# maciejkula/spotlight

Measured on NVIDIA H100. Metric: interactions/sec (BPR MF, 1Mx100Kx64), higher is better.
Workload: dtype f32

## Files before the change

spotlight_b200/csrc/mf.cu:

```cuda
#include <stdlib.h>

#include "segindex.cuh"

namespace {

constexpr int MF_THREADS = 256;

struct MfDev {
    int64_t B;
    int64_t NB;
    int64_t T;
    const int64_t* users; const int64_t* items; const int64_t* negs;
    int32_t loss; int32_t n_neg;
    int64_t U, I; int32_t D;
    float* Wu; float* Wi; float* bu; float* bi;
    float* loss_out; float* pos_out; float* neg_out;
    int32_t* t_a; int32_t* t_b; float* t_g;
    float* partial; int32_t* done;
    int32_t* err;
    SegIndex seg;
    int32_t grad_mode;
    float* dWu; float* dWi; float* dbu; float* dbi;
    int64_t* urows; float* gWu; float* gbu;
    int64_t* irows; float* gWi; float* gbi;
// ... 1076 lines not shown
        SLB_LAUNCH_CHECK("mf_fwd_kernel");
    }
    if (phases & 2) {
        seg_scan_launch(a.seg, a.U, st);
        SLB_LAUNCH_CHECK("seg_scan_kernel");
    }
    int fgrid = static_cast<int>((2 * B + 255) / 256);
    if (fgrid > sms * 8) fgrid = sms * 8;
    if (phases & 4) {
        mf_fill_kernel<<<fgrid, 256, 0, st>>>(a);
        SLB_LAUNCH_CHECK("mf_fill_kernel");
        seg_sort_long_kernel<<<SEG_LONG_CTAS, 256, 0, st>>>(a.seg);
        SLB_LAUNCH_CHECK("seg_sort_long_kernel");
    }
    int64_t bwant = (2 * B + groups - 1) / groups;
    int bgrid = static_cast<int>(bwant < static_cast<int64_t>(sms) * 8 ? bwant : static_cast<int64_t>(sms) * 8);
    const bool bsmall = 2 * B < static_cast<int64_t>(sms) * 24 * 32;
    const int bti = bsmall ? 8 : 32;
    const int64_t tw = ((2 * B + bti - 1) / bti + 3) / 4;
    const int tgrid = static_cast<int>(tw < static_cast<int64_t>(sms) * 16 ? tw : static_cast<int64_t>(sms) * 16);
    const int blpr = lpr;
#define BWD_TILE(MODE)                                                                               \
    if (bsmall) { DISPATCH_LPR3(blpr, mf_bwd_tile_kernel, MODE, 8, tgrid, MF_TILE_THREADS, st, a); } \
    else { DISPATCH_LPR3(blpr, mf_bwd_tile_kernel, MODE, 32, tgrid, MF_TILE_THREADS, st, a); }
    if (x->opt == SLB_OPT_NONE || x->opt == SLB_OPT_ADAM) {
        if (phases & 8) {
            BWD_TILE(0);
            SLB_LAUNCH_CHECK("mf_bwd_tile_kernel");
            launch_long<0>(lpr, st, a);
            SLB_LAUNCH_CHECK("mf_bwd_long_kernel");
        }
        if (x->opt == SLB_OPT_ADAM && (phases & 16)) {
            AdamDev o = {x->beta1, x->beta2, x->one_minus_beta1, x->one_minus_beta2, x->eps, x->weight_decay, x->adam_sched,
                         static_cast<int32_t>(x->adam_step + step_idx)};
            DISPATCH_LPR(lpr, mf_adam_apply_kernel, bgrid, MF_THREADS, st, a, o, x->state2_Wu, x->state2_Wi,
                         x->state2_bu, x->state2_bi, x->last_u, x->last_i);
            SLB_LAUNCH_CHECK("mf_adam_apply_kernel");
        }
    } else {
        if (phases & 8) {
            BWD_TILE(1);
            SLB_LAUNCH_CHECK("mf_bwd_tile_kernel<items>");
            launch_long<1>(lpr, st, a);
            SLB_LAUNCH_CHECK("mf_bwd_long_kernel<items>");
#if BWD_BULK
            if (lpr == 16 && a.D == 64 && !bsmall) {
                auto kern = mf_bwd_tile_kernel<16, 2, 32, true>;
                constexpr int BULK_SMEM = (MF_TILE_THREADS / 32) * 32 * 2 * 256;
                static bool configured = false;
                if (!configured) {
                    cudaFuncSetAttribute(kern, cudaFuncAttributeMaxDynamicSharedMemorySize, BULK_SMEM);
                    configured = true;
                }
                kern<<<tgrid, MF_TILE_THREADS, BULK_SMEM, st>>>(a);
            } else
#endif
            { BWD_TILE(2); }
            SLB_LAUNCH_CHECK("mf_bwd_tile_kernel<users+opt>");
            launch_long<2>(lpr, st, a);
            SLB_LAUNCH_CHECK("mf_bwd_long_kernel<users+opt>");
        }
        if ((phases & 16) && !x->opt_users_only) {
            DISPATCH_LPR2(lpr, mf_apply_kernel, 1, bgrid, MF_THREADS, st, a);
            SLB_LAUNCH_CHECK("mf_apply_kernel<items>");
        }
    }
    return SLB_OK;
}


struct V2Layout {
    PlanDev plan[2];
    StepV2 st;
    size_t bytes;
};

V2Layout v2_layout(void* base, int64_t B, int64_t U, int64_t I, int D) {
    WsCarver ws(base);
    V2Layout l;
    const int64_t R = U + I;
    const int64_t Rpad = (R + SEG_SCAN_TILE - 1) / SEG_SCAN_TILE * SEG_SCAN_TILE;
    l.st.done = ws.take<int32_t>(8);
    int32_t* cnt[2] = {ws.take<int32_t>(Rpad), ws.take<int32_t>(Rpad)};
    for (int k = 0; k < 2; ++k) {
        PlanDev& p = l.plan[k];
        SegIndex& s = p.seg;
        s.R = R;
        s.Rpad = Rpad;
        s.ntiles = s.Rpad / SEG_SCAN_TILE;
        s.Tmax = 3 * B;
        s.cnt = cnt[k];
        s.off = ws.take<int32_t>(s.Rpad);
        s.sid = ws.take<int32_t>(s.Rpad);
        s.status = ws.take<unsigned long long>(s.ntiles);
        s.ticket = ws.take<int32_t>(8);
        s.totals = s.ticket + 4;
        s.seg_row = ws.take<int32_t>(3 * B + 1);
        s.seg_start = ws.take<int32_t>(3 * B + 2);
        s.long_list = ws.take<int32_t>(3 * B / 16 + 2);
        s.members = nullptr; s.long_tmp = nullptr; s.long_bits = nullptr; s.long_words = 0;
        s.long_cap = 0;
        p.mu = ws.take<URec>(B + 1);
        p.mi = ws.take<IRec>(2 * B + 1);
        p.mu_tmp = ws.take<URec>(B + 1);
        p.mi_tmp = ws.take<IRec>(2 * B + 1);
        p.words = (2 * B + 31) / 32;
        p.bits = ws.take<uint32_t>(static_cast<size_t>(SEG_LONG_CTAS) * 2 * p.words);
        p.B = B; p.U = U; p.I = I;
        p.err = nullptr; p.users = nullptr; p.items = nullptr; p.negs = nullptr; p.ratings = nullptr;
    }
    l.st.t_g = ws.take<float>(2 * B);
    l.st.stash = ws.take<float>(static_cast<size_t>(B) * D);
    l.st.partial = ws.take<float>(MF_MAX_GRID);
    l.st.partial_long = ws.take<float>(SEG_LONG_CTAS * 4);
    l.bytes = ws.bytes();
    return l;
}

bool v2_dim_ok(int D) { return D == 8 || D == 16 || D == 32 || D == 64 || D == 128; }

bool v2_eligible(const slb_mf_step_args* x) {
    if (x->fused_workspace == nullptr || x->loss == SLB_LOSS_ADAPTIVE_HINGE || x->opt == SLB_OPT_NONE ||
        x->opt == SLB_OPT_ADAM ||
        !v2_dim_ok(x->dim) || x->pos_out != nullptr || x->neg_out != nullptr)
        return false;
    if (x->opt_users_only) return x->grad_mode == SLB_GRAD_DENSE && x->dWi != nullptr && x->dbi != nullptr;
    return x->grad_mode == SLB_GRAD_COMPACT;
}

int v2_launch_plan(const slb_mf_step_args* x, PlanDev p, int32_t* err, const int64_t* users, const int64_t* items,
                   const int64_t* negs, const float* ratings, int64_t B, cudaStream_t st) {
    p.B = B; p.users = users; p.items = items; p.negs = negs; p.ratings = ratings; p.err = err;
    p.seg.long_cap = seg_sort_cap(lpr_for_dim(x->dim));
    const int sms = slb_sms();
    int g = static_cast<int>((B + 255) / 256);
    if (g > sms * 8) g = sms * 8;
    plan_count_kernel<<<g, 256, 0, st>>>(p);
    SLB_LAUNCH_CHECK("plan_count_kernel");
    seg_scan_launch(p.seg, p.U, st);
    SLB_LAUNCH_CHECK("seg_scan_kernel");
    plan_fill_kernel<<<g, 256, 0, st>>>(p);
    SLB_LAUNCH_CHECK("plan_fill_kernel");
    int64_t tiles = ((3 * B + 31) / 32 + 3) / 4;
    int sg = static_cast<int>(tiles < static_cast<int64_t>(sms) * 16 ? tiles : static_cast<int64_t>(sms) * 16);
    plan_sort_kernel<<<sg, 128, 0, st>>>(p, p.seg.long_cap);
    SLB_LAUNCH_CHECK("plan_sort_kernel");
    plan_order_long_kernel<<<1, 256, 0, st>>>(p);
    SLB_LAUNCH_CHECK("plan_order_long_kernel");
    plan_sort_long_kernel<<<SEG_LONG_CTAS, 256, 0, st>>>(p);
    SLB_LAUNCH_CHECK("plan_sort_long_kernel");
    return SLB_OK;
}

MfDev v2_dev(const slb_mf_step_args* x, int64_t B, float* loss_out) {
    MfDev a = {};
    a.B = B; a.NB = x->norm_batch > 0 ? x->norm_batch : B; a.T = 2 * B;
    a.loss = x->loss; a.n_neg = 1;
    a.U = x->num_users; a.I = x->num_items; a.D = x->dim;
    a.Wu = x->Wu; a.Wi = x->Wi; a.bu = x->bu; a.bi = x->bi;
    a.loss_out = loss_out;
    a.opt = x->opt; a.lr = x->lr; a.wd = x->weight_decay; a.eps = x->eps;
    a.sWu = x->state_Wu; a.sWi = x->state_Wi; a.sbu = x->state_bu; a.sbi = x->state_bi;
    a.frozen_a = -1; a.frozen_b = -1;
    if (x->opt_users_only) { a.dWi = x->dWi; a.dbi = x->dbi; }
    return a;
}

template <int LPR, int LOSS>
void v2_user_launch(const MfDev& a, const PlanDev& p, const StepV2& v, bool small, int grid, cudaStream_t st) {
    const size_t smem = static_cast<size_t>(256 / LPR) * (LPR * 4 + 4) * sizeof(float);
    mf_user_long_kernel<LPR, LOSS><<<SEG_LONG_CTAS * 4, 256, smem, st>>>(a, p, v);
    if (small) mf_user_kernel<LPR, 1, LOSS, 8><<<grid, MF_TILE_THREADS, 0, st>>>(a, p, v, SEG_LONG_CTAS * 4);
    else if (V2_UVPL == 2 && LPR >= 16) {
        mf_user_kernel<LPR / 2, 2, LOSS, 32><<<grid, MF_TILE_THREADS, 0, st>>>(a, p, v, SEG_LONG_CTAS * 4);
    } else mf_user_kernel<LPR, 1, LOSS, 32><<<grid, MF_TILE_THREADS, 0, st>>>(a, p, v, SEG_LONG_CTAS * 4);
}

template <int LPR>
void v2_user_dispatch(const MfDev& a, const PlanDev& p, const StepV2& v, bool small, int grid, cudaStream_t st) {
    switch (a.loss) {
        case SLB_LOSS_POINTWISE: v2_user_launch<LPR, SLB_LOSS_POINTWISE>(a, p, v, small, grid, st); break;
        case SLB_LOSS_BPR: v2_user_launch<LPR, SLB_LOSS_BPR>(a, p, v, small, grid, st); break;
        case SLB_LOSS_REGRESSION: v2_user_launch<LPR, SLB_LOSS_REGRESSION>(a, p, v, small, grid, st); break;
        case SLB_LOSS_POISSON: v2_user_launch<LPR, SLB_LOSS_POISSON>(a, p, v, small, grid, st); break;
        case SLB_LOSS_LOGISTIC: v2_user_launch<LPR, SLB_LOSS_LOGISTIC>(a, p, v, small, grid, st); break;
        default: v2_user_launch<LPR, SLB_LOSS_HINGE>(a, p, v, small, grid, st); break;
    }
}

template <int LPR>
void v2_item_launch(const MfDev& a, const PlanDev& p, const StepV2& v, bool small, int grid, cudaStream_t st) {
    const size_t smem = static_cast<size_t>(256 / LPR) * (LPR * 4 + 4) * sizeof(float);
    mf_item_long_kernel<LPR><<<SEG_LONG_CTAS * 4, 256, smem, st>>>(a, p, v);
    if (small) mf_item_kernel<LPR, 8><<<grid, MF_TILE_THREADS, 0, st>>>(a, p, v);
    else mf_item_kernel<LPR, 32><<<grid, MF_TILE_THREADS, 0, st>>>(a, p, v);
}

int v2_launch_step(const slb_mf_step_args* x, const V2Layout& l, int slot, int32_t* err, const int64_t* users,
                   const int64_t* items, const int64_t* negs, const float* ratings, int64_t B, float* loss_out,
                   cudaStream_t st, int phases) {
    if (phases & 1) {
        const int rc = v2_launch_plan(x, l.plan[slot], err, users, items, negs, ratings, B, st);
        if (rc != SLB_OK) return rc;
    }
    PlanDev p = l.plan[slot];
    p.B = B; p.users = users; p.items = items; p.negs = negs; p.ratings = ratings; p.err = err;
    p.seg.long_cap = seg_sort_cap(lpr_for_dim(x->dim));
    const MfDev a = v2_dev(x, B, loss_out);
    const int sms = slb_sms();
    const int lpr = x->dim / 4;
    if (phases & 2) {
        const bool small = B < static_cast<int64_t>(sms) * 24 * 32;
        const int64_t tw = ((B + (small ? 8 : 32) - 1) / (small ? 8 : 32) + 3) / 4;
        const int grid = static_cast<int>(tw < MF_MAX_GRID ? (tw < 1 ? 1 : tw) : MF_MAX_GRID);
        switch (lpr) {
            case 2: v2_user_dispatch<2>(a, p, l.st, small, grid, st); break;
            case 4: v2_user_dispatch<4>(a, p, l.st, small, grid, st); break;
            case 8: v2_user_dispatch<8>(a, p, l.st, small, grid, st); break;
            case 16: v2_user_dispatch<16>(a, p, l.st, small, grid, st); break;
            default: v2_user_dispatch<32>(a, p, l.st, small, grid, st); break;
        }
        SLB_LAUNCH_CHECK("mf_user_kernel");
    }
    if (phases & 4) {
        const bool small = 2 * B < static_cast<int64_t>(sms) * 24 * 32;
        const int64_t tw = ((2 * B + (small ? 8 : 32) - 1) / (small ? 8 : 32) + 3) / 4;
        const int grid = static_cast<int>(tw < static_cast<int64_t>(sms) * 16 ? (tw < 1 ? 1 : tw) : static_cast<int64_t>(sms) * 16);
        switch (lpr) {
            case 2: v2_item_launch<2>(a, p, l.st, small, grid, st); break;
            case 4: v2_item_launch<4>(a, p, l.st, small, grid, st); break;
            case 8: v2_item_launch<8>(a, p, l.st, small, grid, st); break;
            case 16: v2_item_launch<16>(a, p, l.st, small, grid, st); break;
            default: v2_item_launch<32>(a, p, l.st, small, grid, st); break;
// ... 518 lines not shown
```

spotlight_b200/csrc/mf_v2.cuh:

```cuda
#pragma once

struct __align__(16) URec { int32_t b, i, j, pad; };
struct __align__(8) IRec { int32_t t, useg; };

struct PlanDev {
    SegIndex seg;
    URec* mu;
    IRec* mi;
    URec* mu_tmp;
    IRec* mi_tmp;
    uint32_t* bits;
    int64_t words;
    int32_t* err;
    int64_t B, U, I;
    const int64_t* users; const int64_t* items; const int64_t* negs;
    const float* ratings;
};

struct StepV2 {
    float* t_g;
    float* stash;
    float* partial;
    float* partial_long;
    int32_t* done;
};


__global__ void __launch_bounds__(256) plan_count_kernel(PlanDev p) {
    const int64_t nth = static_cast<int64_t>(gridDim.x) * blockDim.x;
    if (blockIdx.x == 0 && threadIdx.x == 0) p.seg.totals[3] = 0;
    for (int64_t b = static_cast<int64_t>(blockIdx.x) * blockDim.x + threadIdx.x; b < p.B; b += nth) {
        const int64_t u = p.users[b], i = p.items[b], j = p.negs ? p.negs[b] : 0;
        if (u < 0 || u >= p.U || i < 0 || i >= p.I || j < 0 || j >= p.I) { atomicExch(p.err, 1); continue; }
        atomicAdd(p.seg.cnt + u, 1);
        atomicAdd(p.seg.cnt + p.U + i, 1);
        if (p.negs) atomicAdd(p.seg.cnt + p.U + j, 1);
    }
}

__global__ void __launch_bounds__(256) plan_fill_kernel(PlanDev p) {
    const int64_t nth = static_cast<int64_t>(gridDim.x) * blockDim.x;
    const int ubase = p.seg.seg_start[p.seg.totals[2]];
    for (int64_t b = static_cast<int64_t>(blockIdx.x) * blockDim.x + threadIdx.x; b < p.B; b += nth) {
        const int64_t u = p.users[b], i = p.items[b], j = p.negs ? p.negs[b] : 0;
        if (u < 0 || u >= p.U || i < 0 || i >= p.I || j < 0 || j >= p.I) continue;
        const int su = p.seg.off[u] + atomicSub(p.seg.cnt + u, 1) - 1;
        URec r;
        r.b = static_cast<int32_t>(b); r.i = static_cast<int32_t>(i); r.pad = 0;
        r.j = p.negs ? static_cast<int32_t>(j) : __float_as_int(p.ratings[b]);
        p.mu[su] = r;
        const int useg = p.seg.sid[u];
        const int si = p.seg.off[p.U + i] + atomicSub(p.seg.cnt + p.U + i, 1) - 1 - ubase;
        if (!p.negs) {
            IRec a; a.t = static_cast<int32_t>(b); a.useg = useg;
            p.mi[si] = a;
            continue;
        }
        const int sj = p.seg.off[p.U + j] + atomicSub(p.seg.cnt + p.U + j, 1) - 1 - ubase;
        IRec a; a.t = static_cast<int32_t>(2 * b); a.useg = useg;
        IRec c; c.t = static_cast<int32_t>(2 * b + 1); c.useg = useg;
        p.mi[si] = a;
        p.mi[sj] = c;
    }
}

__device__ __forceinline__ int rec_key(const URec& r) { return r.b; }
__device__ __forceinline__ int rec_key(const IRec& r) { return r.t; }

constexpr int PLAN_SORT_SMALL = 16;

__device__ __forceinline__ URec rec_shfl_xor(const URec& r, int j) {
    URec o;
    o.b = __shfl_xor_sync(0xffffffffu, r.b, j); o.i = __shfl_xor_sync(0xffffffffu, r.i, j);
    o.j = __shfl_xor_sync(0xffffffffu, r.j, j); o.pad = 0;
    return o;
}
__device__ __forceinline__ IRec rec_shfl_xor(const IRec& r, int j) {
    IRec o;
    o.t = __shfl_xor_sync(0xffffffffu, r.t, j); o.useg = __shfl_xor_sync(0xffffffffu, r.useg, j);
    return o;
}
__device__ __forceinline__ void rec_set_key(URec& r, int k) { r.b = k; r.i = 0; r.j = 0; r.pad = 0; }
__device__ __forceinline__ void rec_set_key(IRec& r, int k) { r.t = k; r.useg = 0; }

template <typename Rec>
__device__ __forceinline__ void plan_sort_tile(Rec* base, int start, int len, int cap, Rec* tmp_base) {
    const int lane = threadIdx.x & 31;
    if (len == 2) {
        const Rec x = base[start], y = base[start + 1];
        if (rec_key(x) > rec_key(y)) { base[start] = y; base[start + 1] = x; }
    }
    unsigned net = __ballot_sync(0xffffffffu, len > 2 && len <= PLAN_SORT_SMALL);
    const int half = lane >> 4, lid = lane & 15;
    while (net) {
        const int s0 = __ffs(net) - 1;
        net &= net - 1;
        int s1 = -1;
        if (net) { s1 = __ffs(net) - 1; net &= net - 1; }
        const int mine = half == 0 ? s0 : s1;
        const int m_start = __shfl_sync(0xffffffffu, start, mine < 0 ? 0 : mine);
        const int t_len = __shfl_sync(0xffffffffu, len, mine < 0 ? 0 : mine);
        const int m_len = mine < 0 ? 0 : t_len;
        Rec v;
        if (lid < m_len) v = base[m_start + lid];
        else rec_set_key(v, 0x7fffffff);
#pragma unroll
        for (int k = 2; k <= 16; k <<= 1) {
#pragma unroll
            for (int j = k >> 1; j > 0; j >>= 1) {
                const Rec o = rec_shfl_xor(v, j);
                const bool keep_min = ((lid & j) == 0) == ((lid & k) == 0);
                const bool other_smaller = rec_key(o) < rec_key(v);
                if (keep_min == other_smaller) v = o;
            }
        }
        if (lid < m_len) base[m_start + lid] = v;
    }
    unsigned med = __ballot_sync(0xffffffffu, len > PLAN_SORT_SMALL && len <= cap);
    while (med) {
        const int src = __ffs(med) - 1;
        med &= med - 1;
        const int s_start = __shfl_sync(0xffffffffu, start, src);
        const int s_len = __shfl_sync(0xffffffffu, len, src);
        for (int i = lane; i < s_len; i += 32) {
            const Rec x = base[s_start + i];
            int r = 0;
            for (int m = 0; m < s_len; ++m) r += rec_key(base[s_start + m]) < rec_key(x);
            tmp_base[s_start + r] = x;
        }
        __syncwarp();
        for (int i = lane; i < s_len; i += 32) base[s_start + i] = tmp_base[s_start + i];
        __syncwarp();
    }
}

__global__ void __launch_bounds__(128) plan_sort_kernel(PlanDev p, int cap) {
    const int nseg = p.seg.totals[0], nsegA = p.seg.totals[2];
    const int ubase = p.seg.seg_start[nsegA];
    const int lane = threadIdx.x & 31;
    const int ntiles = (nseg + 31) / 32;
    for (int tile = blockIdx.x * 4 + (threadIdx.x >> 5); tile < ntiles; tile += gridDim.x * 4) {
        const int s = tile * 32 + lane;
        int start = 0, len = 0;
        if (s < nseg) { start = p.seg.seg_start[s]; len = p.seg.seg_start[s + 1] - start; }
        plan_sort_tile<URec>(p.mu, start, (s < nsegA) ? len : 0, cap, p.mu_tmp);
        plan_sort_tile<IRec>(p.mi, start - ubase, (s >= nsegA && s < nseg) ? len : 0, cap, p.mi_tmp);
    }
}

template <typename Rec>
__device__ void plan_sort_long_one(Rec* base, Rec* tmp, int start, int len, uint32_t* bits, uint32_t* pre,
                                   int W, uint32_t* sh_scan) {
    const int per = (W + 255) / 256;
    for (int w = threadIdx.x; w < W; w += 256) bits[w] = 0u;
    __syncthreads();
    for (int i = threadIdx.x; i < len; i += 256) {
        const int t = rec_key(base[start + i]);
        atomicOr(bits + (t >> 5), 1u << (t & 31));
    }
    __syncthreads();
    const int lo = threadIdx.x * per, hi = lo + per < W ? lo + per : W;
    uint32_t sum = 0;
    for (int w = lo; w < hi; ++w) sum += __popc(bits[w]);
    sh_scan[threadIdx.x] = sum;
    __syncthreads();
    for (int o = 1; o < 256; o <<= 1) {
        const uint32_t v = threadIdx.x >= o ? sh_scan[threadIdx.x - o] : 0u;
        __syncthreads();
        sh_scan[threadIdx.x] += v;
        __syncthreads();
    }
    uint32_t run = sh_scan[threadIdx.x] - sum;
    for (int w = lo; w < hi; ++w) { pre[w] = run; run += __popc(bits[w]); }
    __syncthreads();
    for (int i = threadIdx.x; i < len; i += 256) {
        const Rec x = base[start + i];
        const int t = rec_key(x);
        const uint32_t r = pre[t >> 5] + __popc(bits[t >> 5] & ((1u << (t & 31)) - 1u));
        tmp[start + r] = x;
    }
    __syncthreads();
    for (int i = threadIdx.x; i < len; i += 256) base[start + i] = tmp[start + i];
    __syncthreads();
}

__global__ void __launch_bounds__(256) plan_order_long_kernel(PlanDev p) {
    __shared__ uint32_t sh_scan[256];
    const int nlong = p.seg.totals[3];
    if (nlong < 2) return;
    uint32_t* bits = p.bits;
    const int W = (p.seg.totals[0] + 31) / 32;
    const int per = (W + 255) / 256;
    for (int w = threadIdx.x; w < W; w += 256) bits[w] = 0u;
    __syncthreads();
    for (int i = threadIdx.x; i < nlong; i += 256) {
        const int s = p.seg.long_list[i];
        atomicOr(bits + (s >> 5), 1u << (s & 31));
    }
    __syncthreads();
    const int lo = threadIdx.x * per, hi = lo + per < W ? lo + per : W;
    uint32_t sum = 0;
    for (int w = lo; w < hi; ++w) sum += __popc(bits[w]);
    sh_scan[threadIdx.x] = sum;
    __syncthreads();
    for (int o = 1; o < 256; o <<= 1) {
        const uint32_t v = threadIdx.x >= o ? sh_scan[threadIdx.x - o] : 0u;
        __syncthreads();
        sh_scan[threadIdx.x] += v;
        __syncthreads();
    }
    uint32_t run = sh_scan[threadIdx.x] - sum;
    for (int w = lo; w < hi; ++w) {
        for (uint32_t m = bits[w]; m; m &= m - 1u) p.seg.long_list[run++] = w * 32 + __ffs(m) - 1;
    }
}

__global__ void __launch_bounds__(256) plan_sort_long_kernel(PlanDev p) {
    __shared__ uint32_t sh_scan[256];
    const int nlong = p.seg.totals[3];
    const int nsegA = p.seg.totals[2];
    const int ubase = p.seg.seg_start[nsegA];
    uint32_t* bits = p.bits + static_cast<size_t>(blockIdx.x) * 2 * p.words;
    uint32_t* pre = bits + p.words;
    for (int li = blockIdx.x; li < nlong; li += gridDim.x) {
        const int s = p.seg.long_list[li];
        const int start = p.seg.seg_start[s];
        const int len = p.seg.seg_start[s + 1] - start;
        if (s < nsegA) plan_sort_long_one<URec>(p.mu, p.mu_tmp, start, len, bits, pre, static_cast<int>((p.B + 31) / 32), sh_scan);
        else plan_sort_long_one<IRec>(p.mi, p.mi_tmp, start - ubase, len, bits, pre, static_cast<int>((2 * p.B + 31) / 32), sh_scan);
    }
}



#ifndef V2_UMINB
#define V2_UMINB 8
#endif
#ifndef V2_UMINB2
#define V2_UMINB2 6
#endif
#ifndef V2_UVPL
#define V2_UVPL 2
#endif
#ifndef V2_UPF
#define V2_UPF 0
#endif

template <int VPL>
struct RowV { float4 v[VPL]; };

template <int LPR, int VPL>
__device__ __forceinline__ RowV<VPL> row_ldg(const float* row, int gl) {
    RowV<VPL> r;
#pragma unroll
    for (int q = 0; q < VPL; ++q) r.v[q] = ldg4(row + gl * 4 + q * LPR * 4);
    return r;
}
template <int LPR, int VPL>
__device__ __forceinline__ RowV<VPL> row_ldcs(const float* row, int gl) {
    RowV<VPL> r;
#pragma unroll
    for (int q = 0; q < VPL; ++q) r.v[q] = __ldcs(reinterpret_cast<const float4*>(row + gl * 4 + q * LPR * 4));
    return r;
}
template <int VPL>
__device__ __forceinline__ RowV<VPL> row_zero() {
    RowV<VPL> r;
#pragma unroll
    for (int q = 0; q < VPL; ++q) r.v[q] = make_float4(0.f, 0.f, 0.f, 0.f);
    return r;
}

template <int LPR, int VPL, int LOSS, bool FULL>
__device__ __forceinline__ void user_member(const RowV<VPL>& w, float ub, const RowV<VPL>& qi, const RowV<VPL>& qj,
                                            float bi_, float bj_, int b, float invB, unsigned gmask, int gl,
                                            float* t_g, RowV<VPL>& acc, float& bacc, bool& nz, float& lsum) {
    if constexpr (LOSS >= SLB_LOSS_REGRESSION) {
        float dp = 0.f;
#pragma unroll
        for (int q = 0; q < VPL; ++q) dp += dot4(w.v[q], qi.v[q]);
        dp = group_sum<LPR>(dp, FULL ? 0xffffffffu : gmask);
        float per, g;
        rating_loss(LOSS, dp + ub + bi_, bj_, per, g);
        g *= invB;
        if (gl == 0) {
            lsum += per;
            t_g[b] = g;
        }
#pragma unroll
        for (int q = 0; q < VPL; ++q) fma4(acc.v[q], g, qi.v[q]);
        bacc += g;
        nz = nz || g != 0.f;
        return;
    }
    float dp = 0.f, dn = 0.f;
#pragma unroll
    for (int q = 0; q < VPL; ++q) { dp += dot4(w.v[q], qi.v[q]); dn += dot4(w.v[q], qj.v[q]); }
    dp = group_sum<LPR>(dp, FULL ? 0xffffffffu : gmask);
    dn = group_sum<LPR>(dn, FULL ? 0xffffffffu : gmask);
    float per, gp, gn;
    pair_loss(LOSS, dp + ub + bi_, dn + ub + bj_, per, gp, gn);
    gp *= invB; gn *= invB;
    if (gl == 0) {
        lsum += per;
        *reinterpret_cast<float2*>(t_g + 2 * static_cast<int64_t>(b)) = make_float2(gp, gn);
    }
#pragma unroll
    for (int q = 0; q < VPL; ++q) { fma4(acc.v[q], gp, qi.v[q]); fma4(acc.v[q], gn, qj.v[q]); }
    bacc += gp + gn;
    nz = nz || gp != 0.f || gn != 0.f;
}

// ... 449 lines not shown
```

spotlight_b200/csrc/segindex.cuh:

```cuda
#pragma once

#include "common.cuh"

constexpr int SEG_SCAN_THREADS = 256;
constexpr int SEG_SCAN_ITEMS = 16;
constexpr int SEG_SCAN_TILE = SEG_SCAN_THREADS * SEG_SCAN_ITEMS;
constexpr int SEG_LONG_CTAS = 8;

struct SegIndex {
    int32_t* cnt;
    int32_t* off;
    int32_t* sid;
    unsigned long long* status;
    int32_t* ticket;
    int32_t* totals;
    int32_t* seg_row;
    int32_t* seg_start;
    int32_t* members;
    int32_t* long_list;
    int32_t* long_tmp;
    uint32_t* long_bits;
    int64_t long_words;
    int32_t long_cap;
    int64_t R;
    int64_t Rpad;
    int64_t ntiles;
    int64_t Tmax;
};

static inline SegIndex seg_index_carve(WsCarver& ws, int64_t R, int64_t Tmax) {
    SegIndex s;
    s.R = R;
    s.Rpad = (R + SEG_SCAN_TILE - 1) / SEG_SCAN_TILE * SEG_SCAN_TILE;
    s.ntiles = s.Rpad / SEG_SCAN_TILE;
    s.Tmax = Tmax;
    s.cnt = ws.take<int32_t>(s.Rpad);
    s.off = ws.take<int32_t>(s.Rpad);
    s.sid = nullptr;
    s.status = ws.take<unsigned long long>(s.ntiles);
    s.ticket = ws.take<int32_t>(8);
    s.totals = s.ticket + 4;
    s.seg_row = ws.take<int32_t>(Tmax + 1);
    s.seg_start = ws.take<int32_t>(Tmax + 2);
    s.members = ws.take<int32_t>(Tmax + 1);
    s.long_list = ws.take<int32_t>(Tmax / 16 + 2);
    s.long_tmp = ws.take<int32_t>(Tmax + 1);
    s.long_words = (Tmax + 31) / 32;
    s.long_bits = ws.take<uint32_t>(static_cast<size_t>(SEG_LONG_CTAS) * 2 * s.long_words);
    s.long_cap = 0;
    return s;
}

#ifdef __CUDACC__

#define SEG_FLAG_AGG 1ull
#define SEG_FLAG_INC 2ull
__device__ __forceinline__ unsigned long long seg_pack(unsigned long long flag, uint32_t sum, uint32_t nz) {
    return (flag << 62) | (static_cast<unsigned long long>(nz) << 31) | sum;
}
__device__ __forceinline__ uint32_t seg_sum(unsigned long long v) { return static_cast<uint32_t>(v & 0x7fffffffull); }
__device__ __forceinline__ uint32_t seg_nz(unsigned long long v) { return static_cast<uint32_t>((v >> 31) & 0x7fffffffull); }
__device__ __forceinline__ unsigned long long seg_flag(unsigned long long v) { return v >> 62; }

static __global__ void __launch_bounds__(SEG_SCAN_THREADS)
seg_tilesum_kernel(SegIndex s) {
    __shared__ unsigned long long sh[SEG_SCAN_THREADS / 32];
    const int64_t base = static_cast<int64_t>(blockIdx.x) * SEG_SCAN_TILE + threadIdx.x * 4;
    unsigned long long part = 0;
#pragma unroll
    for (int i = 0; i < SEG_SCAN_ITEMS / 4; ++i) {
        const int4 v = *reinterpret_cast<const int4*>(s.cnt + base + i * SEG_SCAN_THREADS * 4);
        part += static_cast<unsigned long long>(static_cast<uint32_t>(v.x + v.y + v.z + v.w)) |
                (static_cast<unsigned long long>((v.x != 0) + (v.y != 0) + (v.z != 0) + (v.w != 0)) << 32);
    }
#pragma unroll
    for (int o = 16; o > 0; o >>= 1) part += __shfl_xor_sync(0xffffffffu, part, o);
    if ((threadIdx.x & 31) == 0) sh[threadIdx.x >> 5] = part;
    __syncthreads();
    if (threadIdx.x == 0) {
        unsigned long long tot = 0;
#pragma unroll
        for (int w = 0; w < SEG_SCAN_THREADS / 32; ++w) tot += sh[w];
        s.status[blockIdx.x] = tot;
    }
}

static __global__ void __launch_bounds__(SEG_SCAN_THREADS)
seg_scan_kernel(SegIndex s, int64_t RA) {
    __shared__ uint32_t sh_wsum[SEG_SCAN_THREADS / 32], sh_wnz[SEG_SCAN_THREADS / 32];
    __shared__ unsigned long long sh_part[SEG_SCAN_THREADS / 32];
    __shared__ uint32_t sh_prefix_sum, sh_prefix_nz;
    const int tile = blockIdx.x;
    const int64_t base = static_cast<int64_t>(tile) * SEG_SCAN_TILE + threadIdx.x * SEG_SCAN_ITEMS;
    const int lane = threadIdx.x & 31, warp = threadIdx.x >> 5;

    unsigned long long part = 0;
    for (int j = threadIdx.x; j < tile; j += SEG_SCAN_THREADS) part += s.status[j];

    int32_t c[SEG_SCAN_ITEMS];
#pragma unroll
    for (int i = 0; i < SEG_SCAN_ITEMS / 4; ++i) {
        const int4 v = *reinterpret_cast<const int4*>(s.cnt + base + 4 * i);
        c[4 * i] = v.x; c[4 * i + 1] = v.y; c[4 * i + 2] = v.z; c[4 * i + 3] = v.w;
    }
    uint32_t tsum = 0, tnz = 0;
#pragma unroll
    for (int i = 0; i < SEG_SCAN_ITEMS; ++i) { tsum += c[i]; tnz += c[i] != 0; }

    uint32_t isum = tsum, inz = tnz;
#pragma unroll
    for (int o = 1; o < 32; o <<= 1) {
        const uint32_t a = __shfl_up_sync(0xffffffffu, isum, o);
        const uint32_t b = __shfl_up_sync(0xffffffffu, inz, o);
        if (lane >= o) { isum += a; inz += b; }
    }
#pragma unroll
    for (int o = 16; o > 0; o >>= 1) part += __shfl_xor_sync(0xffffffffu, part, o);
    if (lane == 31) { sh_wsum[warp] = isum; sh_wnz[warp] = inz; }
    if (lane == 0) sh_part[warp] = part;
    __syncthreads();
    uint32_t wsum = 0, wnz = 0;
#pragma unroll
    for (int w = 0; w < SEG_SCAN_THREADS / 32; ++w)
        if (w < warp) { wsum += sh_wsum[w]; wnz += sh_wnz[w]; }
    if (threadIdx.x == 0) {
        unsigned long long tot = 0;
#pragma unroll
        for (int w = 0; w < SEG_SCAN_THREADS / 32; ++w) tot += sh_part[w];
        sh_prefix_sum = static_cast<uint32_t>(tot & 0xffffffffull);
        sh_prefix_nz = static_cast<uint32_t>(tot >> 32);
    }
    __syncthreads();
    uint32_t run = sh_prefix_sum + wsum + isum - tsum;
    uint32_t seg = sh_prefix_nz + wnz + inz - tnz;

#pragma unroll
    for (int i = 0; i < SEG_SCAN_ITEMS; ++i) {
        const int64_t row = base + i;
        if (row == RA) s.totals[2] = static_cast<int32_t>(seg);
        if (c[i] != 0) {
            s.off[row] = static_cast<int32_t>(run);
            if (s.sid) s.sid[row] = static_cast<int32_t>(seg);
            s.seg_row[seg] = static_cast<int32_t>(row);
            s.seg_start[seg] = static_cast<int32_t>(run);
            if (s.long_cap > 0 && c[i] > s.long_cap) s.long_list[atomicAdd(s.totals + 3, 1)] = static_cast<int32_t>(seg);
            run += c[i];
            ++seg;
        }
    }
    if (tile == s.ntiles - 1 && threadIdx.x == SEG_SCAN_THREADS - 1) {
        s.totals[0] = static_cast<int32_t>(seg);
        s.totals[1] = static_cast<int32_t>(run);
        s.seg_start[seg] = static_cast<int32_t>(run);
        if (RA >= s.Rpad) s.totals[2] = static_cast<int32_t>(seg);
    }
}

static __global__ void __launch_bounds__(256) seg_sort_long_kernel(SegIndex s) {
    __shared__ uint32_t sh_scan[256];
    const int nlong = s.totals[3];
    uint32_t* bits = s.long_bits + static_cast<size_t>(blockIdx.x) * 2 * s.long_words;
    uint32_t* pre = bits + s.long_words;
    const int W = static_cast<int>(s.long_words);
    const int per = (W + 255) / 256;
    for (int li = blockIdx.x; li < nlong; li += gridDim.x) {
        const int seg = s.long_list[li];
        const int start = s.seg_start[seg];
        const int len = s.seg_start[seg + 1] - start;
        for (int w = threadIdx.x; w < W; w += 256) bits[w] = 0u;
        __syncthreads();
        for (int i = threadIdx.x; i < len; i += 256) {
            const int t = s.members[start + i];
            atomicOr(bits + (t >> 5), 1u << (t & 31));
        }
        __syncthreads();
        const int lo = threadIdx.x * per, hi = lo + per < W ? lo + per : W;
        uint32_t sum = 0;
        for (int w = lo; w < hi; ++w) sum += __popc(bits[w]);
        sh_scan[threadIdx.x] = sum;
        __syncthreads();
        for (int o = 1; o < 256; o <<= 1) {
            const uint32_t v = threadIdx.x >= o ? sh_scan[threadIdx.x - o] : 0u;
            __syncthreads();
            sh_scan[threadIdx.x] += v;
            __syncthreads();
        }
        uint32_t run = sh_scan[threadIdx.x] - sum;
        for (int w = lo; w < hi; ++w) { pre[w] = run; run += __popc(bits[w]); }
        __syncthreads();
        for (int i = threadIdx.x; i < len; i += 256) {
            const int t = s.members[start + i];
            const uint32_t r = pre[t >> 5] + __popc(bits[t >> 5] & ((1u << (t & 31)) - 1u));
            s.long_tmp[start + r] = t;
        }
        __syncthreads();
        for (int i = threadIdx.x; i < len; i += 256) s.members[start + i] = s.long_tmp[start + i];
        __syncthreads();
    }
}

static inline void seg_scan_launch(const SegIndex& s, int64_t RA, cudaStream_t st) {
    seg_tilesum_kernel<<<static_cast<unsigned>(s.ntiles), SEG_SCAN_THREADS, 0, st>>>(s);
    seg_scan_kernel<<<static_cast<unsigned>(s.ntiles), SEG_SCAN_THREADS, 0, st>>>(s, RA);
}

__device__ __forceinline__ void seg_rearm(const SegIndex& s) {
    const int64_t tid = static_cast<int64_t>(blockIdx.x) * blockDim.x + threadIdx.x;
    const int64_t nth = static_cast<int64_t>(gridDim.x) * blockDim.x;
    (void)nth;
    if (tid == 0 && s.long_cap == 0) s.totals[3] = 0;
}

__device__ __forceinline__ void seg_place(const SegIndex& s, int64_t key, int32_t term) {
    const int32_t old = atomicSub(s.cnt + key, 1);
    s.members[s.off[key] + old - 1] = term;
}

__host__ __device__ constexpr int seg_sort_cap(int G) { return G >= 8 ? 128 : (G >= 4 ? 64 : 16 * G); }

template <int G, typename F>
__device__ __forceinline__ void seg_visit_sorted(const int32_t* __restrict__ members, int start,
                                                 int len, int gl ,
                                                 unsigned gmask, int32_t* sh, F visit,
                                                 bool long_presorted = false) {
    if (len == 1) {
        visit(members[start]);
        return;
    }
    if (len == 2) {
        const int32_t a = members[start], b = members[start + 1];
        visit(a < b ? a : b);
        visit(a < b ? b : a);
        return;
    }
    constexpr int CAP = seg_sort_cap(G);
    if (len <= CAP) {
        int32_t* in = sh;
        int32_t* out = sh + CAP;
        for (int i = gl; i < len; i += G) in[i] = members[start + i];
        __syncwarp(gmask);
        for (int i = gl; i < len; i += G) {
            const int32_t m = in[i];
            int r = 0;
            for (int j = 0; j < len; ++j) r += in[j] < m;
            out[r] = m;
        }
        __syncwarp(gmask);
        for (int i = 0; i < len; ++i) visit(out[i]);
        __syncwarp(gmask);
        return;
    }
    if (long_presorted) {
        for (int i = 0; i < len; ++i) visit(members[start + i]);
        return;
    }
    int32_t last = -1;
    for (int i = 0; i < len; ++i) {
        int32_t best = 0x7fffffff;
        for (int j = gl; j < len; j += G) {
            const int32_t m = members[start + j];
            if (m > last && m < best) best = m;
        }
#pragma unroll
        for (int o = G / 2; o > 0; o >>= 1) {
            const int32_t other = __shfl_xor_sync(gmask, best, o);
            best = other < best ? other : best;
        }
        visit(best);
        last = best;
    }
}

#endif
```

Baseline: 726.3 million.

## Fuse plan scan into single-pass lookback and merge long-segment sort kernels

Replaces the two-kernel tile-sum plus scan with a single-pass decoupled-lookback scan that also writes per-user cursors and zeroes counts. Fill then takes slots with atomicAdd on those cursors instead of atomicSub plus offset lookups. Long-list ordering and status rearm move into the fill kernel, and the long-segment sort is folded into the plan sort kernel, which now stages short segments in shared memory. This cuts kernel launches and global memory traffic in planning, at the cost of lookback spin waits and more shared memory per block.

```diff
diff --git a/spotlight_b200/csrc/mf.cu b/spotlight_b200/csrc/mf.cu
--- a/spotlight_b200/csrc/mf.cu
+++ b/spotlight_b200/csrc/mf.cu
@@ -1182,6 +1182,9 @@
     const int64_t Rpad = (R + SEG_SCAN_TILE - 1) / SEG_SCAN_TILE * SEG_SCAN_TILE;
     l.st.done = ws.take<int32_t>(8);
     int32_t* cnt[2] = {ws.take<int32_t>(Rpad), ws.take<int32_t>(Rpad)};
+    const int64_t ntiles = Rpad / SEG_SCAN_TILE;
+    unsigned long long* status[2] = {ws.take<unsigned long long>(ntiles), ws.take<unsigned long long>(ntiles)};
+    int32_t* ticket[2] = {ws.take<int32_t>(8), ws.take<int32_t>(8)};
     for (int k = 0; k < 2; ++k) {
         PlanDev& p = l.plan[k];
         SegIndex& s = p.seg;
@@ -1192,8 +1195,9 @@
         s.cnt = cnt[k];
         s.off = ws.take<int32_t>(s.Rpad);
         s.sid = ws.take<int32_t>(s.Rpad);
-        s.status = ws.take<unsigned long long>(s.ntiles);
-        s.ticket = ws.take<int32_t>(8);
+        p.ucur = ws.take<unsigned long long>(U);
+        s.status = status[k];
+        s.ticket = ticket[k];
         s.totals = s.ticket + 4;
         s.seg_row = ws.take<int32_t>(3 * B + 1);
         s.seg_start = ws.take<int32_t>(3 * B + 2);
@@ -1237,18 +1241,16 @@
     if (g > sms * 8) g = sms * 8;
     plan_count_kernel<<<g, 256, 0, st>>>(p);
     SLB_LAUNCH_CHECK("plan_count_kernel");
-    seg_scan_launch(p.seg, p.U, st);
-    SLB_LAUNCH_CHECK("seg_scan_kernel");
+    plan_scan_kernel<<<static_cast<unsigned>(p.seg.ntiles), SEG_SCAN_THREADS, 0, st>>>(p);
+    SLB_LAUNCH_CHECK("plan_scan_kernel");
     plan_fill_kernel<<<g, 256, 0, st>>>(p);
     SLB_LAUNCH_CHECK("plan_fill_kernel");
-    int64_t tiles = ((3 * B + 31) / 32 + 3) / 4;
-    int sg = static_cast<int>(tiles < static_cast<int64_t>(sms) * 16 ? tiles : static_cast<int64_t>(sms) * 16);
-    plan_sort_kernel<<<sg, 128, 0, st>>>(p, p.seg.long_cap);
+    const int64_t warps = (3 * B + 31) / 32;
+    const int64_t tiles = (warps + PLAN_SORT_THREADS / 32 - 1) / (PLAN_SORT_THREADS / 32);
+    const int64_t sg_max = static_cast<int64_t>(sms) * 4;
+    const int sg = static_cast<int>(tiles < SEG_LONG_CTAS ? SEG_LONG_CTAS : (tiles < sg_max ? tiles : sg_max));
+    plan_sort_kernel<<<sg, PLAN_SORT_THREADS, 0, st>>>(p, p.seg.long_cap);
     SLB_LAUNCH_CHECK("plan_sort_kernel");
-    plan_order_long_kernel<<<1, 256, 0, st>>>(p);
-    SLB_LAUNCH_CHECK("plan_order_long_kernel");
-    plan_sort_long_kernel<<<SEG_LONG_CTAS, 256, 0, st>>>(p);
-    SLB_LAUNCH_CHECK("plan_sort_long_kernel");
     return SLB_OK;
 }
 
diff --git a/spotlight_b200/csrc/mf_v2.cuh b/spotlight_b200/csrc/mf_v2.cuh
--- a/spotlight_b200/csrc/mf_v2.cuh
+++ b/spotlight_b200/csrc/mf_v2.cuh
@@ -10,6 +10,7 @@
     URec* mu_tmp;
     IRec* mi_tmp;
     uint32_t* bits;
+    unsigned long long* ucur;
     int64_t words;
     int32_t* err;
     int64_t B, U, I;
@@ -38,25 +39,76 @@
     }
 }
 
+struct PlanEmit {
+    int32_t* cnt;
+    unsigned long long* ucur;
+    int64_t U;
+    __device__ __forceinline__ void operator()(int64_t row, int32_t, uint32_t run, uint32_t seg) const {
+        cnt[row] = 0;
+        if (row < U) ucur[row] = (static_cast<unsigned long long>(seg) << 32) | run;
+    }
+};
+
+__global__ void __launch_bounds__(SEG_SCAN_THREADS) plan_scan_kernel(PlanDev p) {
+    seg_scan_tile<true>(p.seg, p.U, PlanEmit{p.seg.cnt, p.ucur, p.U});
+}
+
+__device__ void plan_order_long(const PlanDev& p) {
+    __shared__ uint32_t sh_scan[256];
+    const int nlong = p.seg.totals[3];
+    if (nlong < 2) return;
+    uint32_t* bits = p.bits;
+    const int W = (p.seg.totals[0] + 31) / 32;
+    const int per = (W + 255) / 256;
+    for (int w = threadIdx.x; w < W; w += 256) bits[w] = 0u;
+    __syncthreads();
+    for (int i = threadIdx.x; i < nlong; i += 256) {
+        const int s = p.seg.long_list[i];
+        atomicOr(bits + (s >> 5), 1u << (s & 31));
+    }
+    __syncthreads();
+    const int lo = threadIdx.x * per, hi = lo + per < W ? lo + per : W;
+    uint32_t sum = 0;
+    for (int w = lo; w < hi; ++w) sum += __popc(bits[w]);
+    sh_scan[threadIdx.x] = sum;
+    __syncthreads();
+    for (int o = 1; o < 256; o <<= 1) {
+        const uint32_t v = threadIdx.x >= o ? sh_scan[threadIdx.x - o] : 0u;
+        __syncthreads();
+        sh_scan[threadIdx.x] += v;
+        __syncthreads();
+    }
+    uint32_t run = sh_scan[threadIdx.x] - sum;
+    for (int w = lo; w < hi; ++w) {
+        for (uint32_t m = bits[w]; m; m &= m - 1u) p.seg.long_list[run++] = w * 32 + __ffs(m) - 1;
+    }
+}
+
 __global__ void __launch_bounds__(256) plan_fill_kernel(PlanDev p) {
+    if (blockIdx.x == 0) {
+        plan_order_long(p);
+        seg_lookback_rearm(p.seg);
+    }
     const int64_t nth = static_cast<int64_t>(gridDim.x) * blockDim.x;
     const int ubase = p.seg.seg_start[p.seg.totals[2]];
+    int32_t* icur = p.seg.off + p.U;
     for (int64_t b = static_cast<int64_t>(blockIdx.x) * blockDim.x + threadIdx.x; b < p.B; b += nth) {
         const int64_t u = p.users[b], i = p.items[b], j = p.negs ? p.negs[b] : 0;
         if (u < 0 || u >= p.U || i < 0 || i >= p.I || j < 0 || j >= p.I) continue;
-        const int su = p.seg.off[u] + atomicSub(p.seg.cnt + u, 1) - 1;
+        const unsigned long long cu = atomicAdd(p.ucur + u, 1ull);
+        const int si = atomicAdd(icur + i, 1) - ubase;
+        const int sj = p.negs ? atomicAdd(icur + j, 1) - ubase : 0;
+        const int su = static_cast<int>(cu & 0xffffffffull);
+        const int useg = static_cast<int>(cu >> 32);
         URec r;
         r.b = static_cast<int32_t>(b); r.i = static_cast<int32_t>(i); r.pad = 0;
         r.j = p.negs ? static_cast<int32_t>(j) : __float_as_int(p.ratings[b]);
         p.mu[su] = r;
-        const int useg = p.seg.sid[u];
-        const int si = p.seg.off[p.U + i] + atomicSub(p.seg.cnt + p.U + i, 1) - 1 - ubase;
         if (!p.negs) {
             IRec a; a.t = static_cast<int32_t>(b); a.useg = useg;
             p.mi[si] = a;
             continue;
         }
-        const int sj = p.seg.off[p.U + j] + atomicSub(p.seg.cnt + p.U + j, 1) - 1 - ubase;
         IRec a; a.t = static_cast<int32_t>(2 * b); a.useg = useg;
         IRec c; c.t = static_cast<int32_t>(2 * b + 1); c.useg = useg;
         p.mi[si] = a;
@@ -134,18 +186,37 @@
     }
 }
 
-__global__ void __launch_bounds__(128) plan_sort_kernel(PlanDev p, int cap) {
-    const int nseg = p.seg.totals[0], nsegA = p.seg.totals[2];
-    const int ubase = p.seg.seg_start[nsegA];
+constexpr int PLAN_STAGE_BYTES = 4096;
+constexpr int PLAN_SORT_THREADS = 256;
+
+template <typename Rec>
+__device__ __forceinline__ void plan_stage_sort(Rec* base, int start, int len, int cap, Rec* tmp_base, Rec* sh,
+                                                unsigned char* owner, int2* sh_seg) {
+    constexpr int NREC = PLAN_STAGE_BYTES / static_cast<int>(sizeof(Rec));
     const int lane = threadIdx.x & 31;
-    const int ntiles = (nseg + 31) / 32;
-    for (int tile = blockIdx.x * 4 + (threadIdx.x >> 5); tile < ntiles; tile += gridDim.x * 4) {
-        const int s = tile * 32 + lane;
-        int start = 0, len = 0;
-        if (s < nseg) { start = p.seg.seg_start[s]; len = p.seg.seg_start[s + 1] - start; }
-        plan_sort_tile<URec>(p.mu, start, (s < nsegA) ? len : 0, cap, p.mu_tmp);
-        plan_sort_tile<IRec>(p.mi, start - ubase, (s >= nsegA && s < nseg) ? len : 0, cap, p.mi_tmp);
-    }
+    if (!__any_sync(0xffffffffu, len >= 2)) return;
+    const unsigned some = __ballot_sync(0xffffffffu, len > 0);
+    const int lo = __shfl_sync(0xffffffffu, start, __ffs(some) - 1);
+    const int hi = __shfl_sync(0xffffffffu, start + len, 31 - __clz(some));
+    if (__any_sync(0xffffffffu, len > cap) || hi - lo > NREC) {
+        plan_sort_tile<Rec>(base, start, len, cap, tmp_base);
+        return;
+    }
+    const int n = hi - lo;
+    for (int k = lane; k < n; k += 32) sh[k] = base[lo + k];
+    sh_seg[lane] = make_int2(start - lo, len);
+    for (int k = 0; k < len; ++k) owner[start - lo + k] = static_cast<unsigned char>(lane);
+    __syncwarp();
+    for (int k = lane; k < n; k += 32) {
+        const int2 sg = sh_seg[owner[k]];
+        if (sg.y < 2) continue;
+        const Rec x = sh[k];
+        const int key = rec_key(x);
+        int r = 0;
+        for (int m = sg.x; m < sg.x + sg.y; ++m) r += rec_key(sh[m]) < key;
+        if (sg.x + r != k) base[lo + sg.x + r] = x;
+    }
+    __syncwarp();
 }
 
 template <typename Rec>
@@ -184,50 +255,40 @@
     __syncthreads();
 }
 
-__global__ void __launch_bounds__(256) plan_order_long_kernel(PlanDev p) {
-    __shared__ uint32_t sh_scan[256];
-    const int nlong = p.seg.totals[3];
-    if (nlong < 2) return;
-    uint32_t* bits = p.bits;
-    const int W = (p.seg.totals[0] + 31) / 32;
-    const int per = (W + 255) / 256;
-    for (int w = threadIdx.x; w < W; w += 256) bits[w] = 0u;
-    __syncthreads();
-    for (int i = threadIdx.x; i < nlong; i += 256) {
-        const int s = p.seg.long_list[i];
-        atomicOr(bits + (s >> 5), 1u << (s & 31));
-    }
-    __syncthreads();
-    const int lo = threadIdx.x * per, hi = lo + per < W ? lo + per : W;
-    uint32_t sum = 0;
-    for (int w = lo; w < hi; ++w) sum += __popc(bits[w]);
-    sh_scan[threadIdx.x] = sum;
-    __syncthreads();
-    for (int o = 1; o < 256; o <<= 1) {
-        const uint32_t v = threadIdx.x >= o ? sh_scan[threadIdx.x - o] : 0u;
-        __syncthreads();
-        sh_scan[threadIdx.x] += v;
-        __syncthreads();
-    }
-    uint32_t run = sh_scan[threadIdx.x] - sum;
-    for (int w = lo; w < hi; ++w) {
-        for (uint32_t m = bits[w]; m; m &= m - 1u) p.seg.long_list[run++] = w * 32 + __ffs(m) - 1;
-    }
-}
-
-__global__ void __launch_bounds__(256) plan_sort_long_kernel(PlanDev p) {
-    __shared__ uint32_t sh_scan[256];
-    const int nlong = p.seg.totals[3];
-    const int nsegA = p.seg.totals[2];
+__global__ void __launch_bounds__(PLAN_SORT_THREADS) plan_sort_kernel(PlanDev p, int cap) {
+    constexpr int WARPS = PLAN_SORT_THREADS / 32;
+    __shared__ __align__(16) unsigned char sh_stage[WARPS][PLAN_STAGE_BYTES];
+    __shared__ unsigned char sh_owner[WARPS][PLAN_STAGE_BYTES / sizeof(IRec)];
+    __shared__ int2 sh_seg[WARPS][32];
+    __shared__ uint32_t sh_scan[PLAN_SORT_THREADS];
+    const int nseg = p.seg.totals[0], nsegA = p.seg.totals[2];
     const int ubase = p.seg.seg_start[nsegA];
-    uint32_t* bits = p.bits + static_cast<size_t>(blockIdx.x) * 2 * p.words;
-    uint32_t* pre = bits + p.words;
-    for (int li = blockIdx.x; li < nlong; li += gridDim.x) {
-        const int s = p.seg.long_list[li];
-        const int start = p.seg.seg_start[s];
-        const int len = p.seg.seg_start[s + 1] - start;
-        if (s < nsegA) plan_sort_long_one<URec>(p.mu, p.mu_tmp, start, len, bits, pre, static_cast<int>((p.B + 31) / 32), sh_scan);
-        else plan_sort_long_one<IRec>(p.mi, p.mi_tmp, start - ubase, len, bits, pre, static_cast<int>((2 * p.B + 31) / 32), sh_scan);
+    if (blockIdx.x < SEG_LONG_CTAS) {
+        const int nlong = p.seg.totals[3];
+        uint32_t* bits = p.bits + static_cast<size_t>(blockIdx.x) * 2 * p.words;
+        uint32_t* pre = bits + p.words;
+        for (int li = blockIdx.x; li < nlong; li += SEG_LONG_CTAS) {
+            const int s = p.seg.long_list[li];
+            const int start = p.seg.seg_start[s];
+            const int len = p.seg.seg_start[s + 1] - start;
+            if (s < nsegA) plan_sort_long_one<URec>(p.mu, p.mu_tmp, start, len, bits, pre, static_cast<int>((p.B + 31) / 32), sh_scan);
+            else plan_sort_long_one<IRec>(p.mi, p.mi_tmp, start - ubase, len, bits, pre, static_cast<int>((2 * p.B + 31) / 32), sh_scan);
+        }
+    }
+    const int lane = threadIdx.x & 31, warp = threadIdx.x >> 5;
+    const int ntiles = (nseg + 31) / 32;
+    const int t0 = nsegA / 32;
+    for (int it = blockIdx.x * WARPS + warp; it < ntiles; it += gridDim.x * WARPS) {
+        const int tile = it + t0 < ntiles ? it + t0 : it + t0 - ntiles;
+        const int s = tile * 32 + lane;
+        int start = 0, len = 0;
+        if (s < nseg) { start = p.seg.seg_start[s]; len = p.seg.seg_start[s + 1] - start; }
+        if (tile * 32 < nsegA)
+            plan_stage_sort<URec>(p.mu, start, (s < nsegA) ? len : 0, cap, p.mu_tmp,
+                                  reinterpret_cast<URec*>(sh_stage[warp]), sh_owner[warp], sh_seg[warp]);
+        if (tile * 32 + 32 > nsegA)
+            plan_stage_sort<IRec>(p.mi, start - ubase, (s >= nsegA && s < nseg) ? len : 0, cap, p.mi_tmp,
+                                  reinterpret_cast<IRec*>(sh_stage[warp]), sh_owner[warp], sh_seg[warp]);
     }
 }
 
diff --git a/spotlight_b200/csrc/segindex.cuh b/spotlight_b200/csrc/segindex.cuh
--- a/spotlight_b200/csrc/segindex.cuh
+++ b/spotlight_b200/csrc/segindex.cuh
@@ -66,6 +66,7 @@
 seg_tilesum_kernel(SegIndex s) {
     __shared__ unsigned long long sh[SEG_SCAN_THREADS / 32];
     const int64_t base = static_cast<int64_t>(blockIdx.x) * SEG_SCAN_TILE + threadIdx.x * 4;
+    static_assert(SEG_SCAN_TILE == SEG_SCAN_THREADS * SEG_SCAN_ITEMS, "one tile per CTA");
     unsigned long long part = 0;
 #pragma unroll
     for (int i = 0; i < SEG_SCAN_ITEMS / 4; ++i) {
@@ -85,58 +86,97 @@
     }
 }
 
-static __global__ void __launch_bounds__(SEG_SCAN_THREADS)
-seg_scan_kernel(SegIndex s, int64_t RA) {
-    __shared__ uint32_t sh_wsum[SEG_SCAN_THREADS / 32], sh_wnz[SEG_SCAN_THREADS / 32];
-    __shared__ unsigned long long sh_part[SEG_SCAN_THREADS / 32];
+template <bool LOOKBACK, typename Emit>
+__device__ __forceinline__ void seg_scan_tile(const SegIndex& s, int64_t RA, Emit emit) {
+    constexpr int WARPS = SEG_SCAN_THREADS / 32;
+    constexpr int ROWS_PER_WARP = SEG_SCAN_TILE / WARPS;
+    __shared__ uint32_t sh_wsum[WARPS], sh_wnz[WARPS];
+    __shared__ unsigned long long sh_part[WARPS];
     __shared__ uint32_t sh_prefix_sum, sh_prefix_nz;
-    const int tile = blockIdx.x;
-    const int64_t base = static_cast<int64_t>(tile) * SEG_SCAN_TILE + threadIdx.x * SEG_SCAN_ITEMS;
+    __shared__ int sh_tile;
+    if (LOOKBACK) {
+        if (threadIdx.x == 0) sh_tile = atomicAdd(s.ticket, 1);
+        __syncthreads();
+    }
+    const int tile = LOOKBACK ? sh_tile : static_cast<int>(blockIdx.x);
     const int lane = threadIdx.x & 31, warp = threadIdx.x >> 5;
+    const int64_t base = static_cast<int64_t>(tile) * SEG_SCAN_TILE + warp * ROWS_PER_WARP + lane;
+    const unsigned below = (1u << lane) - 1u;
 
     unsigned long long part = 0;
-    for (int j = threadIdx.x; j < tile; j += SEG_SCAN_THREADS) part += s.status[j];
+    if (!LOOKBACK)
+        for (int j = threadIdx.x; j < tile; j += SEG_SCAN_THREADS) part += s.status[j];
 
     int32_t c[SEG_SCAN_ITEMS];
 #pragma unroll
-    for (int i = 0; i < SEG_SCAN_ITEMS / 4; ++i) {
-        const int4 v = *reinterpret_cast<const int4*>(s.cnt + base + 4 * i);
-        c[4 * i] = v.x; c[4 * i + 1] = v.y; c[4 * i + 2] = v.z; c[4 * i + 3] = v.w;
-    }
+    for (int i = 0; i < SEG_SCAN_ITEMS; ++i) c[i] = s.cnt[base + 32 * i];
     uint32_t tsum = 0, tnz = 0;
 #pragma unroll
     for (int i = 0; i < SEG_SCAN_ITEMS; ++i) { tsum += c[i]; tnz += c[i] != 0; }
-
-    uint32_t isum = tsum, inz = tnz;
-#pragma unroll
-    for (int o = 1; o < 32; o <<= 1) {
-        const uint32_t a = __shfl_up_sync(0xffffffffu, isum, o);
-        const uint32_t b = __shfl_up_sync(0xffffffffu, inz, o);
-        if (lane >= o) { isum += a; inz += b; }
-    }
-#pragma unroll
-    for (int o = 16; o > 0; o >>= 1) part += __shfl_xor_sync(0xffffffffu, part, o);
-    if (lane == 31) { sh_wsum[warp] = isum; sh_wnz[warp] = inz; }
-    if (lane == 0) sh_part[warp] = part;
+#pragma unroll
+    for (int o = 16; o > 0; o >>= 1) {
+        tsum += __shfl_xor_sync(0xffffffffu, tsum, o);
+        tnz += __shfl_xor_sync(0xffffffffu, tnz, o);
+        part += __shfl_xor_sync(0xffffffffu, part, o);
+    }
+    if (lane == 0) { sh_wsum[warp] = tsum; sh_wnz[warp] = tnz; sh_part[warp] = part; }
     __syncthreads();
     uint32_t wsum = 0, wnz = 0;
 #pragma unroll
-    for (int w = 0; w < SEG_SCAN_THREADS / 32; ++w)
+    for (int w = 0; w < WARPS; ++w)
         if (w < warp) { wsum += sh_wsum[w]; wnz += sh_wnz[w]; }
-    if (threadIdx.x == 0) {
+    if (!LOOKBACK && threadIdx.x == 0) {
         unsigned long long tot = 0;
 #pragma unroll
-        for (int w = 0; w < SEG_SCAN_THREADS / 32; ++w) tot += sh_part[w];
+        for (int w = 0; w < WARPS; ++w) tot += sh_part[w];
         sh_prefix_sum = static_cast<uint32_t>(tot & 0xffffffffull);
         sh_prefix_nz = static_cast<uint32_t>(tot >> 32);
     }
+    if (LOOKBACK && warp == 0) {
+        volatile unsigned long long* st = s.status;
+        uint32_t asum = 0, anz = 0;
+#pragma unroll
+        for (int w = 0; w < WARPS; ++w) { asum += sh_wsum[w]; anz += sh_wnz[w]; }
+        if (lane == 0) st[tile] = seg_pack(tile == 0 ? SEG_FLAG_INC : SEG_FLAG_AGG, asum, anz);
+        uint32_t psum = 0, pnz = 0;
+        for (int j = tile - 1; j >= 0;) {
+            const int idx = j - lane;
+            const unsigned long long v = idx >= 0 ? st[idx] : seg_pack(SEG_FLAG_INC, 0u, 0u);
+            if (__any_sync(0xffffffffu, seg_flag(v) == 0)) continue;
+            const unsigned inc = __ballot_sync(0xffffffffu, seg_flag(v) == SEG_FLAG_INC);
+            const int stop = inc ? __ffs(inc) - 1 : 31;
+            uint32_t vs = lane <= stop ? seg_sum(v) : 0u, vn = lane <= stop ? seg_nz(v) : 0u;
+#pragma unroll
+            for (int o = 16; o > 0; o >>= 1) {
+                vs += __shfl_xor_sync(0xffffffffu, vs, o);
+                vn += __shfl_xor_sync(0xffffffffu, vn, o);
+            }
+            psum += vs; pnz += vn;
+            if (inc) break;
+            j -= 32;
+        }
+        if (lane == 0) {
+            if (tile > 0) st[tile] = seg_pack(SEG_FLAG_INC, psum + asum, pnz + anz);
+            sh_prefix_sum = psum;
+            sh_prefix_nz = pnz;
+        }
+    }
     __syncthreads();
-    uint32_t run = sh_prefix_sum + wsum + isum - tsum;
-    uint32_t seg = sh_prefix_nz + wnz + inz - tnz;
+    uint32_t run0 = sh_prefix_sum + wsum;
+    uint32_t seg0 = sh_prefix_nz + wnz;
 
 #pragma unroll
     for (int i = 0; i < SEG_SCAN_ITEMS; ++i) {
-        const int64_t row = base + i;
+        const int64_t row = base + 32 * i;
+        uint32_t isum = static_cast<uint32_t>(c[i]);
+#pragma unroll
+        for (int o = 1; o < 32; o <<= 1) {
+            const uint32_t a = __shfl_up_sync(0xffffffffu, isum, o);
+            if (lane >= o) isum += a;
+        }
+        const unsigned nzm = __ballot_sync(0xffffffffu, c[i] != 0);
+        const uint32_t run = run0 + isum - c[i];
+        const uint32_t seg = seg0 + __popc(nzm & below);
         if (row == RA) s.totals[2] = static_cast<int32_t>(seg);
         if (c[i] != 0) {
             s.off[row] = static_cast<int32_t>(run);
@@ -144,16 +184,26 @@
             s.seg_row[seg] = static_cast<int32_t>(row);
             s.seg_start[seg] = static_cast<int32_t>(run);
             if (s.long_cap > 0 && c[i] > s.long_cap) s.long_list[atomicAdd(s.totals + 3, 1)] = static_cast<int32_t>(seg);
-            run += c[i];
-            ++seg;
-        }
+            emit(row, c[i], run, seg);
+        }
+        run0 += __shfl_sync(0xffffffffu, isum, 31);
+        seg0 += __popc(nzm);
     }
     if (tile == s.ntiles - 1 && threadIdx.x == SEG_SCAN_THREADS - 1) {
-        s.totals[0] = static_cast<int32_t>(seg);
-        s.totals[1] = static_cast<int32_t>(run);
-        s.seg_start[seg] = static_cast<int32_t>(run);
-        if (RA >= s.Rpad) s.totals[2] = static_cast<int32_t>(seg);
-    }
+        s.totals[0] = static_cast<int32_t>(seg0);
+        s.totals[1] = static_cast<int32_t>(run0);
+        s.seg_start[seg0] = static_cast<int32_t>(run0);
+        if (RA >= s.Rpad) s.totals[2] = static_cast<int32_t>(seg0);
+    }
+}
+
+struct SegEmitNone {
+    __device__ __forceinline__ void operator()(int64_t, int32_t, uint32_t, uint32_t) const {}
+};
+
+static __global__ void __launch_bounds__(SEG_SCAN_THREADS)
+seg_scan_kernel(SegIndex s, int64_t RA) {
+    seg_scan_tile<false>(s, RA, SegEmitNone{});
 }
 
 static __global__ void __launch_bounds__(256) seg_sort_long_kernel(SegIndex s) {
@@ -204,6 +254,11 @@
     seg_scan_kernel<<<static_cast<unsigned>(s.ntiles), SEG_SCAN_THREADS, 0, st>>>(s, RA);
 }
 
+__device__ __forceinline__ void seg_lookback_rearm(const SegIndex& s) {
+    for (int64_t t = threadIdx.x; t < s.ntiles; t += blockDim.x) s.status[t] = 0ull;
+    if (threadIdx.x == 0) s.ticket[0] = 0;
+}
+
 __device__ __forceinline__ void seg_rearm(const SegIndex& s) {
     const int64_t tid = static_cast<int64_t>(blockIdx.x) * blockDim.x + threadIdx.x;
     const int64_t nth = static_cast<int64_t>(gridDim.x) * blockDim.x;
```

Result: no change. 744.3 million, median of 6 (+2.5%).
